# Senryoku/zflac

Measured on AMD Instinct MI355X. Metric: Msamples/s decoded (bit-exact) + achieved HBM GB/s, 4096-blk stereo, higher is better.
Workload: dtype int32; 1 GPU; C5 shard: 1250 stereo 16-bit mid/side FLAC streams/GPU x 32 frames x 4096 samples, LPC order 8, partition order 4; streams_total=1250, parallelism=stream-shard x1

## Files before the change

zflac_amd/csrc/decode/pcm_stage.h:

```cpp
#pragma once
#include "lane_reader.h"

namespace zflac {

struct Pend {
    uint4* p;
    uint4 v0, v1;
    __device__ __forceinline__ void flush(bool two) {
        p[0] = v0;
        if (two) p[1] = v1;
    }
};

struct FrameCtx {
    uint64_t out_elem;
    bool write;
    bool packed;
    uint32_t justify;
};

template <int KIND>
__device__ __forceinline__ void store_elem(void* out, uint64_t idx, int32_t v) {
    if constexpr (Kind<KIND>::ESZ == 1) reinterpret_cast<int8_t*>(out)[idx] = (int8_t)v;
    else if constexpr (Kind<KIND>::ESZ == 2) reinterpret_cast<int16_t*>(out)[idx] = (int16_t)v;
    else reinterpret_cast<int32_t*>(out)[idx] = v;
}

__device__ __forceinline__ void pair_values(int32_t v, int32_t& x0, int32_t& x1) {
    const auto r = __builtin_amdgcn_permlane32_swap((uint32_t)v, (uint32_t)v, false, false);
    x0 = (int32_t)r[0];
    x1 = (int32_t)r[1];
}

typedef unsigned short u16x2 __attribute__((ext_vector_type(2)));
typedef short s16x2 __attribute__((ext_vector_type(2)));
__device__ __forceinline__ u16x2 as_u16x2(uint32_t v) { return __builtin_bit_cast(u16x2, v); }
__device__ __forceinline__ uint32_t as_u32(u16x2 v) { return __builtin_bit_cast(uint32_t, v); }
__device__ __forceinline__ uint32_t pk_shl(uint32_t v, uint32_t n) {
    return as_u32(as_u16x2(v) << (u16x2){(unsigned short)n, (unsigned short)n});
}
__device__ __forceinline__ uint32_t pk_sar1(uint32_t v) {
    return as_u32(__builtin_bit_cast(u16x2, __builtin_bit_cast(s16x2, v) >> (s16x2){1, 1}));
}

__device__ __forceinline__ void decorrelate2_ms(uint32_t x0, uint32_t x1, uint32_t& Lp, uint32_t& Rp, uint32_t& ovf) {
    const uint32_t d = pk_sar1(x1);
    const uint32_t r = as_u32(as_u16x2(x0) - as_u16x2(d));
    const uint32_t l = as_u32(as_u16x2(r) + as_u16x2(x1));
    Rp = r;
    Lp = l;
    ovf |= ((x0 ^ d) & (x0 ^ r)) | (~(r ^ x1) & (r ^ l));
}

struct DecMasks {
    uint32_t ms, ls, r1, addl;
    __device__ __forceinline__ void init(uint32_t code) {
        ms = code == 10 ? ~0u : 0u;
        ls = code == 8 ? ~0u : 0u;
        const uint32_t rs = code == 9 ? ~0u : 0u;
        r1 = ~(ms | ls);
        addl = rs | ms;
    }
};

template <int DECOR>
__device__ __forceinline__ void decorrelate2(uint32_t x0, uint32_t x1, const DecMasks& dm, uint32_t& Lp,
                                             uint32_t& Rp, uint32_t& ovf) {
    if constexpr (DECOR == D_MS) {
        decorrelate2_ms(x0, x1, Lp, Rp, ovf);
    } else {
        const uint32_t A = (x0 & ~dm.r1) | (x1 & dm.r1);
        const uint32_t D = (pk_sar1(x1) & dm.ms) | (x1 & dm.ls);
        const uint32_t r = as_u32(as_u16x2(A) - as_u16x2(D));
        const uint32_t E = (r & dm.ms) | (x0 & ~dm.ms);
        const uint32_t F = x1 & dm.addl;
        const uint32_t l = as_u32(as_u16x2(E) + as_u16x2(F));
        Rp = r;
        Lp = l;
        ovf |= ((A ^ D) & (A ^ r)) | (~(E ^ F) & (E ^ l));
    }
}

typedef unsigned int u32x4v __attribute__((ext_vector_type(4)));
typedef __attribute__((address_space(1))) u32x4v guint4;

template <bool MONO>
struct Stage {
    static constexpr uint32_t PIECES = MONO ? 4u : 8u;
    static constexpr uint32_t ROW_FRAMES = 64u / PIECES;
    using Mask = std::conditional_t<MONO, uint64_t, uint32_t>;
    guint4* out;
    __amdgpu_buffer_rsrc_t rs;
    uint32_t gq[4];
    Mask mask;
    uint32_t base;
    uint32_t q0;
    __device__ __forceinline__ static uint32_t lane() { return threadIdx.x & 63u; }
    __device__ __forceinline__ static uint32_t row_frame(int t) {
        return (uint32_t)t * ROW_FRAMES + (lane() / PIECES);
    }
    __device__ __forceinline__ uint32_t quad(uint32_t j, uint32_t p) const {
        if constexpr (MONO) return q0 + j * 4u + (p ^ ((j >> 1) & 3u));
        else return q0 + j * 8u + (p ^ (j & 7u));
    }
    __device__ __forceinline__ void put(uint32_t group, uint4 v) {
        if constexpr (MONO) {
            stage_base()[quad(lane(), group)] = v;
        } else {
            const uint32_t j = lane() & 31u, c = lane() >> 5;
            stage_base()[quad(j, 2u * group + c)] = v;
        }
    }
    __device__ __forceinline__ void read(uint4 (&v)[4]) const {
#pragma unroll
        for (int t = 0; t < 4; t++) v[t] = stage_base()[quad(row_frame(t), lane() & (PIECES - 1u))];
    }
    __device__ __forceinline__ void store(const uint4 (&v)[4], uint4* dummy) const {
        const uint32_t bq = MONO ? base / 8u : base / 4u;
#pragma unroll
        for (int t = 0; t < 4; t++) {
            const bool ok = (mask >> row_frame(t)) & 1u;
            guint4* dst = ok ? out + (gq[t] + bq) : (guint4*)(dummy + (t & 1));
            *dst = __builtin_bit_cast(u32x4v, v[t]);
        }
    }
    __device__ __forceinline__ void store_rsrc(const uint4 (&v)[4]) const {
        const uint32_t bq = MONO ? base / 8u : base / 4u;
        const uint32_t fr = lane() / PIECES;
#pragma unroll
        for (int t = 0; t < 4; t++) {
            const uint32_t dead = (uint32_t)((Mask)~mask >> (t * (int)ROW_FRAMES)) >> fr;
            const uint32_t off = ((gq[t] + bq) << 4) | (dead << 31);
            __builtin_amdgcn_raw_buffer_store_b128(__builtin_bit_cast(u32x4v, v[t]), rs, (int)off, 0, 0);
        }
    }
    template <bool WBR>
    __device__ __forceinline__ void flush(uint4* dummy) {
        uint4 v[4];
        read(v);
        if constexpr (WBR) store_rsrc(v);
        else store(v, dummy);
    }
};
template <int LAY>
using StageOf = Stage<LAY == LAY_MONO>;

__device__ __forceinline__ uint32_t dummy_slot() {
    return 2u * ((threadIdx.x & 63u) + 64u * ((blockIdx.x * DEC_WAVES + (threadIdx.x >> 6)) & 63u));
}

template <int KIND, int LAY, bool WALK, bool WBR>
__device__ __forceinline__ void topup_st(Rdr& rd, Pend& pd, StageOf<LAY>& sg, uint4* dummy) {
    if constexpr (!WALK) {
        if constexpr (staged<KIND, LAY>()) sg.template flush<WBR>(dummy);
        else pd.flush(pend_two<KIND>());
    }
    rd.template topup<topup_quads<KIND>()>();
}

}
```

zflac_amd/csrc/decode/run_subframe.h:

```cpp
#pragma once
#include "chunk.h"

namespace zflac {

#ifdef ZFLAC_PROBE
struct ChunkProbe {
    uint64_t t0, t1, t2;
    uint64_t n[8] = {};
    bool was_fast, was_pair;
    __device__ __forceinline__ void start() {
        was_pair = false;
        t0 = __builtin_amdgcn_s_memtime();
    }
    __device__ __forceinline__ void after_topup() { t1 = __builtin_amdgcn_s_memtime(); }
    __device__ __forceinline__ void pair_chunk(bool pair) { was_pair = pair; }
    __device__ __forceinline__ void after_fast(bool lane_slow) {
        t2 = __builtin_amdgcn_s_memtime();
        was_fast = !__builtin_amdgcn_ballot_w64(lane_slow);
    }
    __device__ __forceinline__ void after_slow(bool redo) {
        const uint64_t t3 = __builtin_amdgcn_s_memtime();
        n[0] += t1 - t0;
        n[1] += t2 - t1;
        n[2] += t3 - t2;
        n[3] += 1;
        n[4] += was_fast ? 1 : 0;
        n[5] += (was_fast && redo) ? 1 : 0;
        n[6] += was_pair ? 1 : 0;
        n[7] += (was_pair && redo) ? 1 : 0;
    }
    __device__ __forceinline__ void finish(void* dummy_base, bool walk) {
        unsigned long long* const out =
            reinterpret_cast<unsigned long long*>(reinterpret_cast<uint8_t*>(dummy_base) + DUMMY_BYTES) + (walk ? 0 : 8);
        if ((threadIdx.x & 63) == 0) {
#pragma unroll
            for (int i = 0; i < 8; i++) atomicAdd(out + i, (unsigned long long)n[i]);
        }
    }
};
#else
struct ChunkProbe {
    __device__ __forceinline__ void start() {}
    __device__ __forceinline__ void after_topup() {}
    __device__ __forceinline__ void pair_chunk(bool) {}
    __device__ __forceinline__ void after_fast(bool) {}
    __device__ __forceinline__ void after_slow(bool) {}
    __device__ __forceinline__ void finish(void*, bool) {}
};
#endif

template <int KIND, int M, int LAY, bool WALK, bool MIX = false, bool WBR = false>
__device__ __forceinline__ void run_subframe(LaneCtx& L, Rdr& rd, const FrameCtx& fc, void* out, int nch, int c,
                                    int32_t c1m, uint32_t bs_max, void* dummy_base, uint32_t out_bytes = 0) {
    static_assert(!WBR || (!WALK && staged<KIND, LAY>()), "only the staged write-back has a resource form");
    constexpr int L_ = CHUNK;
    static_assert(L_ % hist_len<M>() == 0 && L_ % 16 == 0, "a chunk holds whole history rings and output groups");
    uint4* const dummy = reinterpret_cast<uint4*>(dummy_base) + dummy_slot();
    Pend pd;
    pd.p = dummy;
    pd.v0 = pd.v1 = make_uint4(0, 0, 0, 0);
    StageOf<LAY> sg;
    sg.mask = 0;
    sg.base = 0;
    sg.q0 = (threadIdx.x >> 6) * STAGE_QUADS;
    if constexpr (WBR) {
        const uint64_t o = reinterpret_cast<uintptr_t>(out);
        const uint64_t ou = ((uint64_t)(uint32_t)__builtin_amdgcn_readfirstlane((uint32_t)(o >> 32)) << 32) |
                            (uint64_t)(uint32_t)__builtin_amdgcn_readfirstlane((uint32_t)o);
        sg.rs = __builtin_amdgcn_make_buffer_rsrc(reinterpret_cast<void*>(ou), (short)0,
                                                  (int)__builtin_amdgcn_readfirstlane(out_bytes), BUFFER_RSRC_WORD3);
    } else {
        uint64_t outv = reinterpret_cast<uintptr_t>(out);
        asm volatile("" : "+v"(outv));
        sg.out = reinterpret_cast<guint4*>(outv);
    }
    if constexpr (!WALK && staged<KIND, LAY>()) {
#pragma unroll
        for (int t = 0; t < 4; t++)
            sg.gq[t] = (uint32_t)__shfl((int)(uint32_t)(fc.out_elem / 8u), (int)StageOf<LAY>::row_frame(t)) +
                       (StageOf<LAY>::lane() & (StageOf<LAY>::PIECES - 1u));
    }
    Pred<KIND, M> pr;
    if constexpr (WALK) {
        pr.clear();
    } else {
        if (L.mode != M_NONE) parse_subframe<KIND, M>(L, rd, pr);
        else pr.clear();
    }
    const bool need_pack = !WALK && LAY != LAY_MULTI;
    const uint32_t fast_bs = ((!need_pack || fc.packed) && !L.unsafe) ? L.bs : 0u;
    __builtin_amdgcn_s_waitcnt(0);
    uint32_t pair_cool = 0;
    constexpr bool BACKOFF = LAY == LAY_MONO;
    uint32_t pair_fail = 0;
    ChunkProbe probe;
    auto chunk = [&](uint32_t base) __attribute__((always_inline)) {
        probe.start();
        topup_st<KIND, LAY, WALK, WBR>(rd, pd, sg, dummy);
        sg.mask = 0;
        probe.after_topup();
        if (L.mode == M_PRED && base < L.bs && base >= (uint32_t)L.order && L.left == 0 && L.parts_left > 0)
            read_partition_header<KIND>(L, rd);
        if (L.mode != M_NONE && rd.pos() > L.end) set_err(L, rd, E_END_OF_STREAM);
        const bool active = L.mode != M_NONE && base < L.bs;
        uint32_t wu;
        bool lane_fast;
        if constexpr (MIX) {
            wu = base == 0 && L.mode == M_PRED ? (uint32_t)L.order : 0u;
            const bool pred_ok = L.mode == M_PRED && L.left + wu >= (uint32_t)L_ && !L.unsafe;
            const bool cv_ok = L.mode == M_CONST || (L.mode == M_VERB && L.cbps <= 32);
            lane_fast = active && base + L_ <= L.bs && (pred_ok || cv_ok) && (!need_pack || fc.packed);
        } else {
            wu = base == 0 ? (uint32_t)L.order : 0u;
            lane_fast = active && base + L_ <= fast_bs && L.mode == M_PRED && L.left + wu >= (uint32_t)L_;
        }
        const bool need_slow = active && !lane_fast;
        bool redo = __builtin_amdgcn_ballot_w64(need_slow) != 0;
        if (!redo) {
            const uint32_t k_nb = rd.nb;
            const Pred<KIND, M> k_pr = pr;
            if constexpr (!WALK) {
                sg.mask = (typename StageOf<LAY>::Mask)__builtin_amdgcn_ballot_w64(lane_fast && fc.write);
                sg.base = base;
            }
            bool bad = false;
            bool vbad = false;
            uint32_t ovf = 0;
            constexpr auto has = [](auto form) { return decltype(form)::template in_kernel<KIND, LAY, MIX, WALK>(); };
            constexpr bool PAIRS = has(FormPair{});
            const bool pairs = PAIRS && pair_cool == 0 && base != 0 &&
                               __builtin_amdgcn_ballot_w64(lane_fast && (L.k < (WALK ? 1u : 2u) || L.k > PAIR_KMAX ||
                                                                         L.esc)) == 0;
            const bool escs = __builtin_amdgcn_ballot_w64(lane_fast && L.esc) != 0;
            bool wide = false;
            if constexpr (has(FormWide{}))
                wide = __builtin_amdgcn_ballot_w64(lane_fast && L.bps > 30 && L.chan_code >= 8) != 0;
            bool mixed = false;
            if constexpr (has(FormMixed{})) mixed = __builtin_amdgcn_ballot_w64(lane_fast && L.mode != M_PRED) != 0;
            auto all_ms = [&]() {
                bool ms = true;
                if constexpr (LAY == LAY_STEREO) ms = __builtin_amdgcn_ballot_w64(lane_fast && L.chan_code != 10) == 0;
                if constexpr (KIND == 1)
                    ms = ms && __builtin_amdgcn_ballot_w64(lane_fast && (L.wasted != 0 || fc.justify != 0)) == 0;
                return ms;
            };
            auto mono_res = [&]() {
                return has(FormMonoRes{}) && __builtin_amdgcn_ballot_w64(lane_fast && L.k < 2u) == 0;
            };
            auto fast = [&](auto form, uint32_t warm_n = 0) {
                chunk_in_form<KIND, M, L_, LAY, MIX, WALK, decltype(form)>(L, rd, pr, base, fc, out, nch, c, c1m, lane_fast,
                                                                           dummy, bad, pd, sg, vbad, ovf, warm_n);
            };
            auto fast_or_warm = [&](auto form) {
                using Form = decltype(form);
                if (base == 0)
                    chunk_in_form<KIND, M, L_, LAY, MIX, WALK, Warmed<Form>>(L, rd, pr, base, fc, out, nch, c, c1m, lane_fast,
                                                                             dummy, bad, pd, sg, vbad, ovf, wu);
                else
                    chunk_in_form<KIND, M, L_, LAY, MIX, WALK, Form>(L, rd, pr, base, fc, out, nch, c, c1m, lane_fast, dummy,
                                                                     bad, pd, sg, vbad, ovf, wu);
            };
            if (has(FormMixed{}) && mixed) {
                if (wide) fast_or_warm(FormMixedWide{});
                else fast_or_warm(FormMixed{});
            } else if (wide) {
                fast_or_warm(FormWide{});
            } else if (base == 0) {
                fast(FormWarm{}, wu);
            } else if (escs) {
                fast(FormEsc{});
            } else if (!has(FormMsOne{}) || !all_ms()) {
                if (pairs) fast(FormPair{});
                else fast(FormOne{});
            } else if (pairs) {
                fast(FormMsPair{});
            } else if (mono_res()) {
                fast(FormMonoRes{});
            } else {
                fast(FormMsOne{});
            }
            redo = __builtin_amdgcn_ballot_w64(bad && lane_fast) != 0;
            if (PAIRS && pairs && redo) {
                pair_cool = BACKOFF ? 8u << (pair_fail < 4u ? pair_fail : 4u) : 8u;
                pair_fail++;
            } else if (BACKOFF && PAIRS && pairs) {
                pair_fail = 0;
            } else if (pair_cool) {
                pair_cool--;
            }
            pair_cool = __builtin_amdgcn_readfirstlane(pair_cool);
            if constexpr (BACKOFF) pair_fail = __builtin_amdgcn_readfirstlane(pair_fail);
            probe.pair_chunk(PAIRS && pairs && !escs && base != 0);
            if (redo || !lane_fast) {
                rd.nb = k_nb;
            }
            if (redo) {
                pr = k_pr;
                pd.p = dummy;
                sg.mask = 0;
            }
            if (!redo && lane_fast) {
                if (!MIX || L.mode == M_PRED) L.left -= L_ - wu;
                L.dom = L.dom || vbad;
                L.dcr |= ovf & (KIND == 1 ? 0x80008000u : 1u);
            }
        }
        probe.after_fast(need_slow);
        if (redo) slow_chunk<KIND, M, L_, LAY, WALK>(L, rd, pr, base, fc, out, nch, c, c1m);
        probe.after_slow(redo);
    };
    for (uint32_t base = 0; base < bs_max; base += L_) chunk(base);
    probe.finish(dummy_base, WALK);
    if constexpr (!WALK) {
        if constexpr (staged<KIND, LAY>()) {
            sg.template flush<WBR>(dummy);
        } else {
            pd.flush(pend_two<KIND>());
        }
    }
    if (L.mode != M_NONE && rd.pos() > L.end) set_err(L, rd, E_END_OF_STREAM);
}

}
```

Measured before the change: 896,400 Msamples/s.

## Rebuild buffer rsrc per flush, use scalar soffset and cache per-partition ballots

The buffer resource is no longer kept live across the chunk loop. The base pointer and size are held as VGPR words and the descriptor is rebuilt via readfirstlane at each flush, which lowers SGPR pressure. The chunk base moves into the scalar soffset, and dead rows are masked with inverse_ballot on a bit-replicated row mask. For the 16-bit non-mixed kinds, the wave-wide ballots that select the pair, escape and all-mid/side forms are now recomputed only after a partition header or a slow chunk instead of on every chunk. The risk is stale selection state if lane parameters change some other way, plus extra scalar work per flush.

```diff
diff --git a/zflac_amd/csrc/decode/pcm_stage.h b/zflac_amd/csrc/decode/pcm_stage.h
--- a/zflac_amd/csrc/decode/pcm_stage.h
+++ b/zflac_amd/csrc/decode/pcm_stage.h
@@ -1,5 +1,6 @@
 #pragma once
 #include "lane_reader.h"
+#include "row_mask.h"
 
 namespace zflac {
 
@@ -90,7 +91,7 @@
     static constexpr uint32_t ROW_FRAMES = 64u / PIECES;
     using Mask = std::conditional_t<MONO, uint64_t, uint32_t>;
     guint4* out;
-    __amdgpu_buffer_rsrc_t rs;
+    uint32_t rw[3];
     uint32_t gq[4];
     Mask mask;
     uint32_t base;
@@ -124,21 +125,24 @@
             *dst = __builtin_bit_cast(u32x4v, v[t]);
         }
     }
-    __device__ __forceinline__ void store_rsrc(const uint4 (&v)[4]) const {
-        const uint32_t bq = MONO ? base / 8u : base / 4u;
-        const uint32_t fr = lane() / PIECES;
+    __device__ __forceinline__ void store_rsrc(const uint4 (&v)[4], uint32_t sbase) {
+        const uint32_t so = MONO ? sbase * 2u : sbase * 4u;
+        asm volatile("" : "+v"(rw[0]), "+v"(rw[1]), "+v"(rw[2]));
+        const uint64_t o = ((uint64_t)(uint32_t)__builtin_amdgcn_readfirstlane(rw[1]) << 32) |
+                           (uint64_t)(uint32_t)__builtin_amdgcn_readfirstlane(rw[0]);
+        const __amdgpu_buffer_rsrc_t rs = __builtin_amdgcn_make_buffer_rsrc(
+            reinterpret_cast<void*>(o), (short)0, (int)__builtin_amdgcn_readfirstlane(rw[2]), BUFFER_RSRC_WORD3);
 #pragma unroll
         for (int t = 0; t < 4; t++) {
-            const uint32_t dead = (uint32_t)((Mask)~mask >> (t * (int)ROW_FRAMES)) >> fr;
-            const uint32_t off = ((gq[t] + bq) << 4) | (dead << 31);
-            __builtin_amdgcn_raw_buffer_store_b128(__builtin_bit_cast(u32x4v, v[t]), rs, (int)off, 0, 0);
+            const uint32_t off = __builtin_amdgcn_inverse_ballot_w64(row_lane_mask<MONO>(mask, t)) ? gq[t] : 0x80000000u;
+            __builtin_amdgcn_raw_buffer_store_b128(__builtin_bit_cast(u32x4v, v[t]), rs, (int)off, (int)so, 0);
         }
     }
     template <bool WBR>
-    __device__ __forceinline__ void flush(uint4* dummy) {
+    __device__ __forceinline__ void flush(uint4* dummy, uint32_t sbase) {
         uint4 v[4];
         read(v);
-        if constexpr (WBR) store_rsrc(v);
+        if constexpr (WBR) store_rsrc(v, sbase);
         else store(v, dummy);
     }
 };
@@ -150,9 +154,9 @@
 }
 
 template <int KIND, int LAY, bool WALK, bool WBR>
-__device__ __forceinline__ void topup_st(Rdr& rd, Pend& pd, StageOf<LAY>& sg, uint4* dummy) {
+__device__ __forceinline__ void topup_st(Rdr& rd, Pend& pd, StageOf<LAY>& sg, uint4* dummy, uint32_t sbase) {
     if constexpr (!WALK) {
-        if constexpr (staged<KIND, LAY>()) sg.template flush<WBR>(dummy);
+        if constexpr (staged<KIND, LAY>()) sg.template flush<WBR>(dummy, sbase);
         else pd.flush(pend_two<KIND>());
     }
     rd.template topup<topup_quads<KIND>()>();
diff --git a/zflac_amd/csrc/decode/row_mask.h b/zflac_amd/csrc/decode/row_mask.h
--- /dev/null
+++ b/zflac_amd/csrc/decode/row_mask.h
@@ -0,0 +1,32 @@
+#pragma once
+#include <cstdint>
+
+#if !defined(__HIPCC__) && !defined(__host__)
+#define __host__
+#define __device__
+#endif
+
+namespace zflac {
+
+#if defined(__HIP_DEVICE_COMPILE__)
+__device__ uint64_t s_bitreplicate(uint32_t x) __asm("llvm.amdgcn.s.bitreplicate");
+#endif
+
+__host__ __device__ constexpr uint64_t double_bits(uint32_t x) {
+#if defined(__HIP_DEVICE_COMPILE__)
+    if (!__builtin_is_constant_evaluated()) return s_bitreplicate(x);
+#endif
+    uint64_t r = 0;
+    for (int i = 0; i < 32; i++) r |= (uint64_t)((x >> i) & 1u) * 3u << (2 * i);
+    return r;
+}
+
+template <bool MONO>
+__host__ __device__ constexpr uint64_t row_lane_mask(uint64_t frames, int t) {
+    constexpr int ROW_FRAMES = MONO ? 16 : 8;
+    const uint32_t row = (uint32_t)(frames >> (t * ROW_FRAMES)) & ((1u << ROW_FRAMES) - 1u);
+    if constexpr (MONO) return double_bits((uint32_t)double_bits(row));
+    else return double_bits((uint32_t)double_bits((uint32_t)double_bits(row)));
+}
+
+}
diff --git a/zflac_amd/csrc/decode/run_subframe.h b/zflac_amd/csrc/decode/run_subframe.h
--- a/zflac_amd/csrc/decode/run_subframe.h
+++ b/zflac_amd/csrc/decode/run_subframe.h
@@ -65,10 +65,9 @@
     sg.q0 = (threadIdx.x >> 6) * STAGE_QUADS;
     if constexpr (WBR) {
         const uint64_t o = reinterpret_cast<uintptr_t>(out);
-        const uint64_t ou = ((uint64_t)(uint32_t)__builtin_amdgcn_readfirstlane((uint32_t)(o >> 32)) << 32) |
-                            (uint64_t)(uint32_t)__builtin_amdgcn_readfirstlane((uint32_t)o);
-        sg.rs = __builtin_amdgcn_make_buffer_rsrc(reinterpret_cast<void*>(ou), (short)0,
-                                                  (int)__builtin_amdgcn_readfirstlane(out_bytes), BUFFER_RSRC_WORD3);
+        sg.rw[0] = (uint32_t)o;
+        sg.rw[1] = (uint32_t)(o >> 32);
+        sg.rw[2] = out_bytes;
     } else {
         uint64_t outv = reinterpret_cast<uintptr_t>(out);
         asm volatile("" : "+v"(outv));
@@ -79,6 +78,10 @@
         for (int t = 0; t < 4; t++)
             sg.gq[t] = (uint32_t)__shfl((int)(uint32_t)(fc.out_elem / 8u), (int)StageOf<LAY>::row_frame(t)) +
                        (StageOf<LAY>::lane() & (StageOf<LAY>::PIECES - 1u));
+        if constexpr (WBR) {
+#pragma unroll
+            for (int t = 0; t < 4; t++) sg.gq[t] <<= 4;
+        }
     }
     Pred<KIND, M> pr;
     if constexpr (WALK) {
@@ -93,14 +96,23 @@
     uint32_t pair_cool = 0;
     constexpr bool BACKOFF = LAY == LAY_MONO;
     uint32_t pair_fail = 0;
+    constexpr bool HOLD = WALK || (KIND == 1 && !MIX && M != 32);
+    auto count = [](bool p) { return (uint32_t)__builtin_popcountll(__builtin_amdgcn_ballot_w64(p)); };
+    uint32_t sel_stale = 1, k_bad = 0, esc_n = 0, ms_bad = 0;
+    if constexpr (HOLD && FormMsOne::template in_kernel<KIND, LAY, MIX, WALK>()) {
+        if constexpr (LAY == LAY_STEREO) ms_bad = count(L.mode != M_NONE && L.chan_code != 10);
+        if constexpr (KIND == 1) ms_bad += count(L.mode != M_NONE && (L.wasted != 0 || fc.justify != 0));
+    }
     ChunkProbe probe;
     auto chunk = [&](uint32_t base) __attribute__((always_inline)) {
         probe.start();
-        topup_st<KIND, LAY, WALK, WBR>(rd, pd, sg, dummy);
+        topup_st<KIND, LAY, WALK, WBR>(rd, pd, sg, dummy, base - (uint32_t)L_);
         sg.mask = 0;
         probe.after_topup();
-        if (L.mode == M_PRED && base < L.bs && base >= (uint32_t)L.order && L.left == 0 && L.parts_left > 0)
-            read_partition_header<KIND>(L, rd);
+        const bool part_hdr =
+            L.mode == M_PRED && base < L.bs && base >= (uint32_t)L.order && L.left == 0 && L.parts_left > 0;
+        if constexpr (HOLD) sel_stale += count(part_hdr);
+        if (part_hdr) read_partition_header<KIND>(L, rd);
         if (L.mode != M_NONE && rd.pos() > L.end) set_err(L, rd, E_END_OF_STREAM);
         const bool active = L.mode != M_NONE && base < L.bs;
         uint32_t wu;
@@ -128,16 +140,27 @@
             uint32_t ovf = 0;
             constexpr auto has = [](auto form) { return decltype(form)::template in_kernel<KIND, LAY, MIX, WALK>(); };
             constexpr bool PAIRS = has(FormPair{});
-            const bool pairs = PAIRS && pair_cool == 0 && base != 0 &&
-                               __builtin_amdgcn_ballot_w64(lane_fast && (L.k < (WALK ? 1u : 2u) || L.k > PAIR_KMAX ||
-                                                                         L.esc)) == 0;
-            const bool escs = __builtin_amdgcn_ballot_w64(lane_fast && L.esc) != 0;
+            bool pairs, escs;
+            if constexpr (HOLD) {
+                if (sel_stale) {
+                    sel_stale = 0;
+                    k_bad = count(lane_fast && (L.k < (WALK ? 1u : 2u) || L.k > PAIR_KMAX || L.esc));
+                    esc_n = count(lane_fast && L.esc);
+                }
+                pairs = PAIRS && pair_cool == 0 && base != 0 && k_bad == 0;
+                escs = esc_n != 0;
+            } else {
+                pairs = PAIRS && pair_cool == 0 && base != 0 &&
+                        __builtin_amdgcn_ballot_w64(lane_fast && (L.k < (WALK ? 1u : 2u) || L.k > PAIR_KMAX || L.esc)) == 0;
+                escs = __builtin_amdgcn_ballot_w64(lane_fast && L.esc) != 0;
+            }
             bool wide = false;
             if constexpr (has(FormWide{}))
                 wide = __builtin_amdgcn_ballot_w64(lane_fast && L.bps > 30 && L.chan_code >= 8) != 0;
             bool mixed = false;
             if constexpr (has(FormMixed{})) mixed = __builtin_amdgcn_ballot_w64(lane_fast && L.mode != M_PRED) != 0;
             auto all_ms = [&]() {
+                if constexpr (HOLD) return ms_bad == 0;
                 bool ms = true;
                 if constexpr (LAY == LAY_STEREO) ms = __builtin_amdgcn_ballot_w64(lane_fast && L.chan_code != 10) == 0;
                 if constexpr (KIND == 1)
@@ -206,14 +229,17 @@
             }
         }
         probe.after_fast(need_slow);
-        if (redo) slow_chunk<KIND, M, L_, LAY, WALK>(L, rd, pr, base, fc, out, nch, c, c1m);
+        if (redo) {
+            slow_chunk<KIND, M, L_, LAY, WALK>(L, rd, pr, base, fc, out, nch, c, c1m);
+            if constexpr (HOLD) sel_stale = 1;
+        }
         probe.after_slow(redo);
     };
     for (uint32_t base = 0; base < bs_max; base += L_) chunk(base);
     probe.finish(dummy_base, WALK);
     if constexpr (!WALK) {
         if constexpr (staged<KIND, LAY>()) {
-            sg.template flush<WBR>(dummy);
+            sg.template flush<WBR>(dummy, __builtin_amdgcn_readfirstlane(sg.base));
         } else {
             pd.flush(pend_two<KIND>());
         }
```

Result: faster. 910,700 Msamples/s, median of 6 (+1.6%).
